# User-tian/Conan

Hardware: AMD Instinct MI355X
Metric: chunks/sec (80 ms chunk, 16 kHz), all streams summed; p50 per-chunk latency beside it (higher is better)
Workload: dtype f32 (3×bf16-limb products, f32 accumulate)

## Files before the change

### conan_amd/csrc/resblock_limb.hip

```cpp
#include <algorithm>
#include <cstring>
#include <type_traits>

#include "kernels.h"

#define RL_MAX_SLOTS 256

#ifndef RL_HELPER_PRIO
#define RL_HELPER_PRIO 3
#endif
#ifndef RL_MATRIX_PRIO
#define RL_MATRIX_PRIO 0
#endif
#ifndef RL_STAMPS
#define RL_STAMPS 0
#endif

#ifdef RL_ABLATE_W
#define RL_WOFF(x) 0
#define RL_WOFF2(a_, b_) (b_)
#else
#define RL_WOFF(x) (x)
#define RL_WOFF2(a_, b_) (a_)
#endif

namespace cnk {

namespace {

typedef float f32x4 __attribute__((ext_vector_type(4)));
typedef __bf16 bf16x8 __attribute__((ext_vector_type(8)));
typedef unsigned short u16;
typedef const f32x4 __attribute__((address_space(1)))* gcf4;
typedef f32x4 __attribute__((address_space(1)))* gf4;
typedef const float __attribute__((address_space(1)))* gcf1;
typedef const int __attribute__((address_space(1)))* gci;

__device__ __forceinline__ f32x4 rl_gload(const void* p) { return *(gcf4)(p); }
__device__ __forceinline__ float4 rl_gload4(const float* p) { const f32x4 v = *(gcf4)(p); return make_float4(v[0], v[1], v[2], v[3]); }
__device__ __forceinline__ void rl_gstore4(float* p, const float4 v) { *(gf4)(p) = (f32x4){v.x, v.y, v.z, v.w}; }

typedef float f32x2 __attribute__((ext_vector_type(2)));
typedef __bf16 bf16x2 __attribute__((ext_vector_type(2)));
__device__ __forceinline__ void rl_split2(const f32x2 x, unsigned& h, unsigned& m, unsigned& l) {
  h = __builtin_bit_cast(unsigned, __builtin_convertvector(x, bf16x2));
  const f32x2 hf = {__uint_as_float(h << 16), __uint_as_float(h & 0xffff0000u)};
  const f32x2 r1 = x - hf;
  m = __builtin_bit_cast(unsigned, __builtin_convertvector(r1, bf16x2));
  const f32x2 mf = {__uint_as_float(m << 16), __uint_as_float(m & 0xffff0000u)};
  const f32x2 r2 = r1 - mf;
  l = __builtin_bit_cast(unsigned, __builtin_convertvector(r2, bf16x2));
}
__device__ __forceinline__ f32x2 rl_lrelu2(const f32x2 x, const float slope) {
  const f32x2 sx = x * slope;
  return (f32x2){__builtin_fmaxf(x[0], sx[0]), __builtin_fmaxf(x[1], sx[1])};
}

template <int C_, int NR2_, int SPAN_>
struct RLGeom {
  static constexpr int C = C_, NR2 = NR2_;
  static constexpr int NR1 = NR2 + 1;
  static constexpr int RO = 16 * NR2;
  static constexpr int XT_ROWS = 16 * NR1;
  static constexpr int MAXSPAN = SPAN_;
  static constexpr int WR_MAX = XT_ROWS + MAXSPAN;
  static constexpr int LDB = C + 16;
  static constexpr int PLW = WR_MAX * LDB;
  static constexpr int PLX = XT_ROWS * LDB;
  static constexpr int LDA = C + 4;
  static constexpr int LDS_U16 = 3 * (PLW + PLX);
  static constexpr int NCT = C / 16;
  static constexpr int NCW = C == 64 ? 1 : 2;
  static constexpr int RSPLIT = 4 / (NCT / NCW);
  static constexpr int NRW1 = (NR1 + RSPLIT - 1) / RSPLIT;
  static constexpr int NRW2 = (NR2 + RSPLIT - 1) / RSPLIT;
  static constexpr int KB = C / 32;
  static constexpr int RING = 2;
  static constexpr int C4 = C / 4;
  static constexpr int BLK = 3 * 512;
  static_assert(C % 32 == 0 && NCT % NCW == 0 && 4 % (NCT / NCW) == 0 && (KB == 1 || KB % RING == 0), "channel count");
  static_assert(RO * LDA * 4 <= 3 * PLX * 2, "accumulator image inside the xt planes");
  static_assert(LDS_U16 * 2 + 32 + 8 * RL_MAX_SLOTS <= 160 * 1024, "LDS budget");
};

template <int NCW, int RING>
__device__ __forceinline__ void rl_prefetch_w(f32x4 (&bw)[RING][NCW][3], const u16* __restrict__ wl, const long long ct_stride) {
#pragma unroll
  for (int q = 0; q < RING; ++q) {
#pragma unroll
    for (int c = 0; c < NCW; ++c)
#pragma unroll
      for (int p = 0; p < 3; ++p) bw[q][c][p] = rl_gload(wl + c * ct_stride + q * 1536 + p * 512);
    __builtin_amdgcn_sched_barrier(0);
  }
}

template <int NRW, int NCW, int LDB, int KB, int RING>
__device__ __forceinline__ void rl_gemm(const u16* __restrict__ src, const int plane, const int row0, const int tap_stride, const int k,
                                        const u16* __restrict__ wl, const long long ct_stride, const u16* __restrict__ wl_next,
                                        const long long ct_stride_next, f32x4 (&acc)[NRW][NCW], f32x4 (&bw)[RING][NCW][3], const int lane) {
  const u16* abase = src + (row0 + (lane & 15)) * LDB + 8 * (lane >> 4);
  f32x4 af[NRW][3];
#pragma unroll
  for (int r = 0; r < NRW; ++r)
#pragma unroll
    for (int p = 0; p < 3; ++p) af[r][p] = *reinterpret_cast<const f32x4*>(abase + p * plane + r * 16 * LDB);
  const int tstep = tap_stride * LDB;
  if constexpr (KB == 1) {
    static_assert(RING == 2, "ring");
    constexpr int PA[6] = {2, 1, 0, 1, 0, 0}, PB[6] = {0, 1, 2, 0, 1, 0};
    auto block = [&](const int j, auto slot_c) __attribute__((always_inline)) {
      constexpr int SL = decltype(slot_c)::value;
      const u16* anext = abase + (j + 1) * tstep;
#pragma unroll
      for (int s = 0; s < 6; ++s)
#pragma unroll
        for (int r = 0; r < NRW; ++r) {
#pragma unroll
          for (int c = 0; c < NCW; ++c)
            acc[r][c] = __builtin_amdgcn_mfma_f32_16x16x32_bf16(__builtin_bit_cast(bf16x8, bw[SL][c][PB[s]]), __builtin_bit_cast(bf16x8, af[r][PA[s]]), acc[r][c], 0, 0, 0);
#ifndef RL_ABLATE_A
          if (s == 0) af[r][2] = *reinterpret_cast<const f32x4*>(anext + 2 * plane + r * 16 * LDB);
          if (s == 3) af[r][1] = *reinterpret_cast<const f32x4*>(anext + plane + r * 16 * LDB);
          if (s == 5) af[r][0] = *reinterpret_cast<const f32x4*>(anext + r * 16 * LDB);
#endif
        }
      const bool own = j + 2 < k;
      const u16* wsrc = own ? wl + (long long)(j + 2) * 1536 : wl_next + (long long)(j + 2 - k) * 1536;
      const long long cs = own ? ct_stride : ct_stride_next;
#pragma unroll
      for (int c = 0; c < NCW; ++c)
#pragma unroll
        for (int p = 0; p < 3; ++p) bw[SL][c][p] = rl_gload(wsrc + c * cs + p * 512);
#pragma unroll
      for (int s = 0; s < 6; ++s) {
        if (s == 0 || s == 3 || s == 5) {
#pragma unroll
          for (int r = 0; r < NRW; ++r) {
            __builtin_amdgcn_sched_group_barrier(0x008, NCW, 0);
            __builtin_amdgcn_sched_group_barrier(0x100, 1, 0);
          }
        } else {
          __builtin_amdgcn_sched_group_barrier(0x008, NRW * NCW, 0);
        }
      }
      __builtin_amdgcn_sched_group_barrier(0x020, 3 * NCW, 0);
    };
    int j = 0;
    for (; j + 1 < k; j += 2) {
      block(j, std::integral_constant<int, 0>{});
      block(j + 1, std::integral_constant<int, 1>{});
    }
    if (j < k) {
      block(j, std::integral_constant<int, 0>{});
#pragma unroll
      for (int c = 0; c < NCW; ++c)
#pragma unroll
        for (int p = 0; p < 3; ++p) { const f32x4 t = bw[0][c][p]; bw[0][c][p] = bw[1][c][p]; bw[1][c][p] = t; }
    }
    return;
  }
  for (int j = 0; j < k; ++j) {
    const u16* arow = abase + j * tstep;
    const bool last = j + 1 == k;
    const u16* wnext = last ? wl_next : wl + (long long)(j + 1) * KB * 1536;
    const long long cnext = last ? ct_stride_next : ct_stride;
#pragma unroll
    for (int q = 0; q < KB; ++q) {
      const u16* anext = (q + 1 < KB) ? arow + (q + 1) * 32 : arow + tstep;
      constexpr int PA[6] = {2, 1, 0, 1, 0, 0}, PB[6] = {0, 1, 2, 0, 1, 0};
#pragma unroll
      for (int s = 0; s < 6; ++s)
#pragma unroll
        for (int r = 0; r < NRW; ++r) {
#pragma unroll
          for (int c = 0; c < NCW; ++c)
            acc[r][c] = __builtin_amdgcn_mfma_f32_16x16x32_bf16(__builtin_bit_cast(bf16x8, bw[q % RING][c][PB[s]]), __builtin_bit_cast(bf16x8, af[r][PA[s]]),
                                                                acc[r][c], 0, 0, 0);
#ifndef RL_ABLATE_A
          if (s == 0) af[r][2] = *reinterpret_cast<const f32x4*>(anext + 2 * plane + r * 16 * LDB);
          if (s == 3) af[r][1] = *reinterpret_cast<const f32x4*>(anext + plane + r * 16 * LDB);
          if (s == 5) af[r][0] = *reinterpret_cast<const f32x4*>(anext + r * 16 * LDB);
#endif
        }
      if (q + RING < KB) {
#pragma unroll
        for (int c = 0; c < NCW; ++c)
#pragma unroll
          for (int p = 0; p < 3; ++p) bw[q % RING][c][p] = rl_gload(wl + RL_WOFF(((long long)j * KB + q + RING) * 1536) + c * ct_stride + p * 512);
      } else {
#pragma unroll
        for (int c = 0; c < NCW; ++c)
#pragma unroll
          for (int p = 0; p < 3; ++p) bw[q % RING][c][p] = rl_gload(RL_WOFF2(wnext, wl) + (q + RING - KB) * 1536 + c * cnext + p * 512);
      }
#pragma unroll
      for (int s = 0; s < 6; ++s) {
        if (s == 0 || s == 3 || s == 5) {
#pragma unroll
          for (int r = 0; r < NRW; ++r) {
            __builtin_amdgcn_sched_group_barrier(0x008, NCW, 0);
            __builtin_amdgcn_sched_group_barrier(0x100, 1, 0);
          }
        } else {
          __builtin_amdgcn_sched_group_barrier(0x008, NRW * NCW, 0);
        }
      }
      __builtin_amdgcn_sched_group_barrier(0x020, 3 * NCW, 0);
      __builtin_amdgcn_sched_barrier(0);
    }
  }
}

}

#define RL_SEL(br_, f) ((br_) == 0 ? a.p[0].f : ((br_) == 1 ? a.p[1].f : a.p[2].f))

template <int C, int NR2, int SPAN, bool MERGE>
__global__ __launch_bounds__(512, 2) void resblock_limb_kernel(const RBArgs a) {
  using G = RLGeom<C, NR2, SPAN>;
  constexpr int LDB = G::LDB;
  __shared__ __attribute__((aligned(16))) u16 lds[G::LDS_U16 + 16 + 4 * RL_MAX_SLOTS];
  u16* const win = lds;
  u16* const xt = lds + 3 * G::PLW;
  float* const accimg = reinterpret_cast<float*>(xt);
  int* const meta = reinterpret_cast<int*>(lds + G::LDS_U16);
  int* const sptab = meta + 8;
  const int tid = threadIdx.x;
  const int lane = tid & 63;
  const int wave = __builtin_amdgcn_readfirstlane(tid >> 6);
  const int ntiles = a.ntiles;
  const float slope = a.slope;
  const int T = a.T;
  constexpr bool merge = MERGE;
  const int np = a.nprob;

  if (wave >= 4) {
    const int ht = tid - 256;
    __builtin_amdgcn_s_setprio(RL_HELPER_PRIO);
    auto hbar = [&]() __attribute__((always_inline)) { asm volatile("s_waitcnt lgkmcnt(0)\n\ts_barrier" ::: "memory"); };
    constexpr int NIT = (G::WR_MAX * G::C4 + 255) / 256;
    float4 wv[NIT];
    int wtotal = 0, wzr = 0;
    auto win_issue = [&](const int p, const int i, const int t0, const int slot, const int pos) __attribute__((always_inline)) {
      const int k = RL_SEL(p, k), d = RL_SEL(p, dil);
      const int wr = G::XT_ROWS + (k - 1) * d;
      const int tw0 = t0 - (k - 1) - (k - 1) * d;
      const int xmode = a.p[0].x.mode, xrate = a.p[0].x.rate;
      const float* xb = RL_SEL(p, x.base) + (long long)(xmode == 0 ? slot : i) * RL_SEL(p, x.slot_stride);
      const unsigned rbase = (xmode == 0 ? (unsigned)pos * (unsigned)xrate : 0u) + (unsigned)(RL_SEL(p, x.off) + tw0);
      const unsigned rmask = xmode == 0 ? (unsigned)RL_SEL(p, x.lmask) : 0xffffffffu;
      wtotal = wr * G::C4;
#pragma unroll
      for (int u = 0; u < NIT; ++u) {
        const int idx = ht + 256 * u;
        const int w = idx / G::C4, c4 = idx - w * G::C4;
        const unsigned row = (rbase + (unsigned)w) & rmask;
        wv[u] = idx < wtotal ? rl_gload4(xb + (long long)row * C + c4 * 4) : make_float4(0.f, 0.f, 0.f, 0.f);
      }
      const long long abs0 = (xmode == 0 ? (long long)pos * xrate : 0ll) + t0 - (k - 1);
      wzr = abs0 >= 0 ? 0 : (abs0 < -(long long)G::XT_ROWS ? G::XT_ROWS : (int)-abs0);
    };
    auto win_write = [&]() __attribute__((always_inline)) {
#pragma unroll
      for (int u = 0; u < NIT; ++u) {
        const int idx = ht + 256 * u;
        const int w = idx / G::C4, c4 = idx - w * G::C4;
        unsigned h[2], m[2], l[2];
        rl_split2(rl_lrelu2((f32x2){wv[u].x, wv[u].y}, slope), h[0], m[0], l[0]);
        rl_split2(rl_lrelu2((f32x2){wv[u].z, wv[u].w}, slope), h[1], m[1], l[1]);
        if (idx < wtotal) {
          u16* dst = win + w * LDB + c4 * 4;
          *reinterpret_cast<uint2*>(dst) = make_uint2(h[0], h[1]);
          *reinterpret_cast<uint2*>(dst + G::PLW) = make_uint2(m[0], m[1]);
          *reinterpret_cast<uint2*>(dst + 2 * G::PLW) = make_uint2(l[0], l[1]);
        }
      }
      if (ht == 0) meta[0] = wzr;
    };
    constexpr int NOUT = (G::RO * G::C4) / 256;
    static_assert((G::RO * G::C4) % 256 == 0 && 256 % G::C4 == 0, "output tile / helper threads");
    const int oc4 = ht % G::C4;
    float4 oacc[NOUT], ores[NOUT], osum[MERGE ? NOUT : 1], ob2 = make_float4(0.f, 0.f, 0.f, 0.f);
    const float* oxb = nullptr; const float* ob2p = nullptr;
    float* oyb = nullptr;
    unsigned oyr0 = 0, oym = 0, oxr0 = 0, oxm = 0;
    int ot0 = 0, op = 0, oyC = C;
#pragma unroll
    for (int u = 0; u < (MERGE ? NOUT : 1); ++u) osum[u] = make_float4(0.f, 0.f, 0.f, 0.f);
    auto out_fetch = [&](const int p, const int i, const int t0, const int slot, const int pos) __attribute__((always_inline)) {
      const int xmode = a.p[0].x.mode, xrate = a.p[0].x.rate, ymode = a.p[0].y.mode, yrate = a.p[0].y.rate;
      oxb = RL_SEL(p, x.base) + (long long)(xmode == 0 ? slot : i) * RL_SEL(p, x.slot_stride);
      oxr0 = (xmode == 0 ? (unsigned)pos * (unsigned)xrate : 0u) + (unsigned)(RL_SEL(p, x.off) + t0);
      oxm = xmode == 0 ? (unsigned)RL_SEL(p, x.lmask) : 0xffffffffu;
      if (!merge) {
        oyb = RL_SEL(p, y.base) + (long long)(ymode == 0 ? slot : i) * RL_SEL(p, y.slot_stride);
        oyr0 = (ymode == 0 ? (unsigned)pos * (unsigned)yrate : 0u) + (unsigned)(RL_SEL(p, y.off) + t0);
        oym = ymode == 0 ? (unsigned)RL_SEL(p, y.lmask) : 0xffffffffu;
      } else {
        const int mmode = a.ymean.mode;
        oyb = a.ymean.base + (long long)(mmode == 0 ? slot : i) * a.ymean.slot_stride;
        oyr0 = (mmode == 0 ? (unsigned)pos * (unsigned)a.ymean.rate : 0u) + (unsigned)(a.ymean.off + t0);
        oym = mmode == 0 ? (unsigned)a.ymean.lmask : 0xffffffffu;
        oyC = a.ymean.C;
      }
      ot0 = t0; op = p;
      ob2p = RL_SEL(p, b2) + oc4 * 4;
#pragma unroll
      for (int u = 0; u < NOUT; ++u) oacc[u] = *reinterpret_cast<const float4*>(accimg + ((ht + 256 * u) / G::C4) * G::LDA + oc4 * 4);
      ob2 = rl_gload4(ob2p);
#pragma unroll
      for (int u = 0; u < NOUT; ++u) {
        const int r = (ht + 256 * u) / G::C4;
        ores[u] = ot0 + r < T ? rl_gload4(oxb + (long long)((oxr0 + (unsigned)r) & oxm) * C + oc4 * 4) : make_float4(0.f, 0.f, 0.f, 0.f);
      }
    };
    auto out_store = [&]() __attribute__((always_inline)) {
#pragma unroll
      for (int u = 0; u < NOUT; ++u) {
        const int r = (ht + 256 * u) / G::C4;
        if (ot0 + r < T) {
          const float4 v = make_float4((oacc[u].x + ob2.x) + ores[u].x, (oacc[u].y + ob2.y) + ores[u].y, (oacc[u].z + ob2.z) + ores[u].z, (oacc[u].w + ob2.w) + ores[u].w);
          if constexpr (!MERGE) rl_gstore4(oyb + (long long)((oyr0 + (unsigned)r) & oym) * C + oc4 * 4, v);
          else {
            float4 sm = osum[MERGE ? u : 0];
            if (op == 0) sm = v; else { sm.x += v.x; sm.y += v.y; sm.z += v.z; sm.w += v.w; }
            osum[MERGE ? u : 0] = sm;
            if (op == np - 1) {
              const float dn = (float)np;
              if (np > 1) { sm.x /= dn; sm.y /= dn; sm.z /= dn; sm.w /= dn; }
              sm.x = sm.x > 0.f ? sm.x : sm.x * slope; sm.y = sm.y > 0.f ? sm.y : sm.y * slope;
              sm.z = sm.z > 0.f ? sm.z : sm.z * slope; sm.w = sm.w > 0.f ? sm.w : sm.w * slope;
              rl_gstore4(oyb + (long long)((oyr0 + (unsigned)r) & oym) * oyC + oc4 * 4, sm);
            }
          }
        }
      }
    };
#if RL_STAMPS
    const unsigned long long h_t0 = __builtin_amdgcn_s_memtime();
    unsigned long long h_t[6] = {0, 0, 0, 0, 0, 0};
#define RL_HT(i_) h_t[i_] = __builtin_amdgcn_s_memtime() - h_t0
#else
#define RL_HT(i_)
#endif
    int dv0 = 0;
    if (wave == 4 && lane == 0) dv0 = __hip_atomic_fetch_add(a.sched, 1, __ATOMIC_RELAXED, __HIP_MEMORY_SCOPE_AGENT);
    for (int e = ht; e < a.n; e += 256) {
      const int sl = a.slots ? *(gci)(a.slots + e) : e;
      sptab[2 * e] = sl; sptab[2 * e + 1] = a.pos ? *(gci)(a.pos + sl) : 0;
    }
    const int tps = a.tiles_per_slot, per_prob = a.n * tps;
    auto decode = [&](const int e, int& p, int& i, int& t0) __attribute__((always_inline)) {
      if constexpr (!MERGE) {
        const int b = e / per_prob, rem = e - b * per_prob;
        p = b == 0 ? a.order[0] : (b == 1 ? a.order[1] : a.order[2]);
        i = rem / tps; t0 = (rem - i * tps) * G::RO;
      } else {
        const int g = e / np;
        p = e - g * np; i = g / tps; t0 = (g - i * tps) * G::RO;
      }
    };
    int cur = -1, p = -1, i = 0, t0 = 0;
    if (wave == 4) {
      cur = __builtin_amdgcn_readfirstlane(dv0) * (merge ? np : 1);
      if (cur >= ntiles) cur = -1;
      if (cur >= 0) decode(cur, p, i, t0);
      if (lane == 0) { meta[1] = cur; meta[2] = p; meta[3] = 0; }
    }
    RL_HT(0);
    asm volatile("s_waitcnt lgkmcnt(0)\n\ts_barrier" ::: "memory");
    RL_HT(1);
    if (wave != 4) {
      cur = __builtin_amdgcn_readfirstlane(meta[1]);
      if (cur >= 0) decode(cur, p, i, t0);
    }
    if (cur >= 0) {
    int slot = __builtin_amdgcn_readfirstlane(sptab[2 * i]), pos = __builtin_amdgcn_readfirstlane(sptab[2 * i + 1]);
    win_issue(p, i, t0, slot, pos);
    RL_HT(2);
    int gen = 1;
    int dv = 0, dnext = -1;
    auto draw_issue = [&](const int have, const int idx_prev, const int p_prev) __attribute__((always_inline)) {
      if (wave == 4 && lane == 0 && have) {
        if (merge && p_prev != np - 1) dnext = idx_prev + 1;
        else { dnext = -1; dv = __hip_atomic_fetch_add(a.sched, 1, __ATOMIC_RELAXED, __HIP_MEMORY_SCOPE_AGENT); }
      }
    };
    auto draw_take = [&](const int have) __attribute__((always_inline)) {
      int idx = -1;
      if (!have) return idx;
      if (wave == 4) {
        const int drawn = dv * (merge ? np : 1);
        idx = __builtin_amdgcn_readfirstlane(dnext >= 0 ? dnext : drawn);
        if (idx >= ntiles) idx = -1;
        if (lane == 0) {
          meta[1] = idx;
          asm volatile("s_waitcnt lgkmcnt(0)" ::: "memory");
          __hip_atomic_store(&meta[3], gen, __ATOMIC_RELEASE, __HIP_MEMORY_SCOPE_WORKGROUP);
        }
      } else {
        while (__hip_atomic_load(&meta[3], __ATOMIC_ACQUIRE, __HIP_MEMORY_SCOPE_WORKGROUP) != gen) __builtin_amdgcn_s_sleep(4);
        idx = __builtin_amdgcn_readfirstlane(meta[1]);
      }
      ++gen;
      return idx;
    };
    const bool deep = ntiles >= 5 * (int)gridDim.x * (merge ? np : 1);
    auto stage = [&](const int e) __attribute__((always_inline)) {
      int pe, ie, te;
      decode(e, pe, ie, te);
      win_issue(pe, ie, te, __builtin_amdgcn_readfirstlane(sptab[2 * ie]), __builtin_amdgcn_readfirstlane(sptab[2 * ie + 1]));
      return pe;
    };
    int nxt = -1, pn = -1;
    if (deep) {
      draw_issue(1, cur, p);
      nxt = draw_take(1);
    }
    RL_HT(3);
    win_write();
    RL_HT(4);
    hbar();
    RL_HT(5);
#if RL_STAMPS
    if (a.dbg && blockIdx.x == 0 && wave == 4 && lane == 0) { unsigned long long* q = a.dbg + 256 * 4 + 12; for (int e = 0; e < 6; ++e) q[e] = h_t[e]; }
#endif
    bool pending = false;
    for (;;) {
      const bool have = deep ? nxt >= 0 : true;
      if (deep && nxt >= 0) pn = stage(nxt);
      draw_issue(have, deep ? nxt : cur, deep ? pn : p);
      if (pending) out_store();
      int nn = -1;
      if (!deep) {
        nxt = draw_take(have); pn = -1;
        if (nxt >= 0) pn = stage(nxt);
      }
      if (ht == 0) meta[2] = nxt >= 0 ? pn : -1;
      hbar();
      hbar();
      if (nxt >= 0) win_write();
      hbar();
      hbar();
      out_fetch(p, i, t0, slot, pos);
      pending = true;
      if (deep) nn = draw_take(have);
      if (nxt < 0) break;
      cur = nxt;
      decode(cur, p, i, t0);
      slot = __builtin_amdgcn_readfirstlane(sptab[2 * i]); pos = __builtin_amdgcn_readfirstlane(sptab[2 * i + 1]);
      nxt = nn;
    }
    if (pending) out_store();
    }
    if (ht == 0) {
      const int d = __hip_atomic_fetch_add(a.sched + 1, 1, __ATOMIC_RELAXED, __HIP_MEMORY_SCOPE_AGENT);
      if (d == (int)gridDim.x - 1) {
        __hip_atomic_store(a.sched, 0, __ATOMIC_RELAXED, __HIP_MEMORY_SCOPE_AGENT);
        __hip_atomic_store(a.sched + 1, 0, __ATOMIC_RELAXED, __HIP_MEMORY_SCOPE_AGENT);
      }
    }
    return;
  }

  if (RL_MATRIX_PRIO) __builtin_amdgcn_s_setprio(RL_MATRIX_PRIO);
  auto bar = [&]() __attribute__((always_inline)) { asm volatile("s_waitcnt lgkmcnt(0)\n\ts_barrier" ::: "memory"); };
  const int wc = wave % (4 / G::RSPLIT);
  const int wr = wave / (4 / G::RSPLIT);
  const int ct0 = wc * G::NCW;
  const int lr = lane & 15, lg = lane >> 4;
#if RL_STAMPS
  unsigned long long st_gemm = 0, st_t0 = __builtin_amdgcn_s_memtime(), st_r0 = __builtin_amdgcn_s_memrealtime(), st_bar = 0, st_b3 = 0, st_b1 = 0, st_b4 = 0, st_b2 = 0, st_e1 = 0, st_e2 = 0, st_tiles = 0, st_head = 0, st_pre = 0, st_mid = 0;
#define RL_T() __builtin_amdgcn_s_memtime()
#define RL_BAR(acc_) do { const unsigned long long q0_ = RL_T(); bar(); const unsigned long long q1_ = RL_T(); acc_ += q1_ - q0_; st_bar += q1_ - q0_; } while (0)
#define RL_GEMM(...) do { const unsigned long long s0_ = RL_T(); __VA_ARGS__; asm volatile("s_nop 0" ::"v"(acc[0][0][0])); st_gemm += RL_T() - s0_; } while (0)
#else
#define RL_BAR(acc_) bar()
#define RL_GEMM(...) __VA_ARGS__
#endif
  f32x4 bw[G::RING][G::NCW][3];
  bar();
  int p = __builtin_amdgcn_readfirstlane(meta[2]);
  if (p < 0) return;
  {
    const long long cs = (long long)(RL_SEL(p, k) + 1) * G::KB * G::BLK;
    rl_prefetch_w<G::NCW, G::RING>(bw, RL_SEL(p, w1l) + (long long)ct0 * cs + lane * 8, cs);
  }
  bar();
#if RL_STAMPS
  st_head = RL_T() - st_t0;
#endif
  while (p >= 0) {
#if RL_STAMPS
    const unsigned long long top_ = RL_T();
#endif
    const int k = RL_SEL(p, k), d = RL_SEL(p, dil);
    const u16* const w1 = RL_SEL(p, w1l);
    const u16* const w2 = RL_SEL(p, w2l);
    const float* const b1 = RL_SEL(p, b1);
    const long long ct_stride = (long long)(k + 1) * G::KB * G::BLK;
    const int zrows = __builtin_amdgcn_readfirstlane(meta[0]);
    f32x4 b1v[G::NCW];
#pragma unroll
    for (int c = 0; c < G::NCW; ++c) b1v[c] = rl_gload(b1 + (ct0 + c) * 16 + 4 * lg);
    int pn;
    {
      f32x4 acc[G::NRW1][G::NCW];
#pragma unroll
      for (int r = 0; r < G::NRW1; ++r)
#pragma unroll
        for (int c = 0; c < G::NCW; ++c) acc[r][c] = (f32x4){0.f, 0.f, 0.f, 0.f};
      const int rt0 = wr * G::NRW1;
#if RL_STAMPS
      st_pre += RL_T() - top_;
#endif
      RL_GEMM(rl_gemm<G::NRW1, G::NCW, LDB, G::KB, G::RING>(win, G::PLW, rt0 * 16, d, k, w1 + (long long)ct0 * ct_stride + lane * 8, ct_stride,
                                                           w2 + (long long)ct0 * ct_stride + lane * 8, ct_stride, acc, bw, lane));
      RL_BAR(st_b3);
#if RL_STAMPS
      const unsigned long long e1_0 = RL_T();
#endif
      auto epilogue1 = [&](auto zr_c) __attribute__((always_inline)) {
        constexpr bool ZR = decltype(zr_c)::value;
#pragma unroll
        for (int c = 0; c < G::NCW; ++c) {
          const int col = (ct0 + c) * 16 + 4 * lg;
#pragma unroll
          for (int r = 0; r < G::NRW1; ++r) {
            if (rt0 + r < G::NR1) {
              const int m = (rt0 + r) * 16 + lr;
              unsigned h[2], mm[2], l[2];
              const f32x4 v = acc[r][c] + b1v[c];
              rl_split2(rl_lrelu2((f32x2){v[0], v[1]}, slope), h[0], mm[0], l[0]);
              rl_split2(rl_lrelu2((f32x2){v[2], v[3]}, slope), h[1], mm[1], l[1]);
              const bool zr = ZR && m < zrows;
              u16* dst = xt + m * LDB + col;
              *reinterpret_cast<uint2*>(dst) = zr ? make_uint2(0u, 0u) : make_uint2(h[0], h[1]);
              *reinterpret_cast<uint2*>(dst + G::PLX) = zr ? make_uint2(0u, 0u) : make_uint2(mm[0], mm[1]);
              *reinterpret_cast<uint2*>(dst + 2 * G::PLX) = zr ? make_uint2(0u, 0u) : make_uint2(l[0], l[1]);
            }
          }
        }
      };
      if (zrows > 0) epilogue1(std::true_type{}); else epilogue1(std::false_type{});
#if RL_STAMPS
      asm volatile("s_waitcnt lgkmcnt(0)" ::: "memory"); st_e1 += RL_T() - e1_0; ++st_tiles;
#endif
    }
    RL_BAR(st_b1);
#if RL_STAMPS
    const unsigned long long mid_ = RL_T();
#endif
    pn = __builtin_amdgcn_readfirstlane(meta[2]);
    const int pnx = pn >= 0 ? pn : p;
    const long long csn = (long long)(RL_SEL(pnx, k) + 1) * G::KB * G::BLK;
    const u16* const w1n = RL_SEL(pnx, w1l) + (long long)ct0 * csn + lane * 8;
    {
      f32x4 acc[G::NRW2][G::NCW];
#pragma unroll
      for (int r = 0; r < G::NRW2; ++r)
#pragma unroll
        for (int c = 0; c < G::NCW; ++c) acc[r][c] = (f32x4){0.f, 0.f, 0.f, 0.f};
      const int rt0 = wr * G::NRW2;
#if RL_STAMPS
      st_mid += RL_T() - mid_;
#endif
      RL_GEMM(rl_gemm<G::NRW2, G::NCW, LDB, G::KB, G::RING>(xt, G::PLX, rt0 * 16, 1, k, w2 + (long long)ct0 * ct_stride + lane * 8, ct_stride,
                                                           w1n, csn, acc, bw, lane));
      RL_BAR(st_b4);
#if RL_STAMPS
      const unsigned long long e2_0 = RL_T();
#endif
#pragma unroll
      for (int c = 0; c < G::NCW; ++c) {
        const int col = (ct0 + c) * 16 + 4 * lg;
#pragma unroll
        for (int r = 0; r < G::NRW2; ++r) {
          if (rt0 + r < NR2) *reinterpret_cast<f32x4*>(accimg + ((rt0 + r) * 16 + lr) * G::LDA + col) = acc[r][c];
        }
      }
#if RL_STAMPS
      asm volatile("s_waitcnt lgkmcnt(0)" ::: "memory"); st_e2 += RL_T() - e2_0;
#endif
    }
    RL_BAR(st_b2);
    p = pn;
  }
#if RL_STAMPS
  if (a.dbg && tid == 0) {
    unsigned long long* o = a.dbg + blockIdx.x * 4;
    if (blockIdx.x == 0) { unsigned long long* q = a.dbg + 256 * 4; q[0] = st_b3; q[1] = st_b1; q[2] = st_b4; q[3] = st_b2; q[4] = st_e1; q[5] = st_e2; q[6] = st_tiles; q[7] = st_gemm; q[8] = __builtin_amdgcn_s_memtime() - st_t0; q[9] = st_head; q[10] = st_pre; q[11] = st_mid; }
    o[0] = st_gemm; o[1] = __builtin_amdgcn_s_memtime() - st_t0; o[2] = __builtin_amdgcn_s_memrealtime() - st_r0; o[3] = st_bar;
  }
#endif
}


namespace {
struct RLCand { int C, NR2, span; };
const RLCand kLimbCands[] = {{32, 10, 50}, {64, 5, 50}, {128, 2, 50}};
}

bool resblock_limb_supported(int C, int kmax, int span_max) {
  for (const RLCand& c : kLimbCands)
    if (c.C == C && span_max <= c.span) return kmax <= 16;
  return false;
}

int resblock_limb_rows(int C, int span_max) {
  int best = 0;
  for (const RLCand& c : kLimbCands)
    if (c.C == C && span_max <= c.span) best = std::max(best, 16 * c.NR2);
  return best;
}

template <int C, int NR2, int SPAN, bool MERGE = false>
static bool launch_rl(const RBArgs& ain, int num_cu, hipStream_t st) {
  RBArgs a = ain;
  const int ro = 16 * NR2;
  a.tiles_per_slot = (a.T + ro - 1) / ro;
  const int total = a.nprob * a.n * a.tiles_per_slot;
  if (total <= 0) return true;
  if (!a.sched) return false;
  for (int p = 0; p < a.nprob; ++p) if (!a.p[p].w1l || !a.p[p].w2l) return false;
  if (a.n > RL_MAX_SLOTS) return false;
  if (!(a.slope > 0.f && a.slope <= 1.f)) return false;
  for (int p = 0; p < 3; ++p) a.order[p] = p;
  std::stable_sort(a.order, a.order + a.nprob, [&](int x, int y) { return a.p[x].k > a.p[y].k; });
  const int grid = std::min(a.merge ? total / a.nprob : total, num_cu);
  a.tiles = nullptr; a.ntiles = total;
  hipLaunchKernelGGL((resblock_limb_kernel<C, NR2, SPAN, MERGE>), dim3(grid), dim3(512), 0, st, a);
  return true;
}

bool launch_resblock_limb(const RBArgs& a, int C, int rows, int num_cu, hipStream_t st) {
  const int nr2 = rows / 16;
  if (a.merge) {
    if (C == 32 && nr2 == 10) return launch_rl<32, 10, 50, true>(a, num_cu, st);
    if (C == 64 && nr2 == 5) return launch_rl<64, 5, 50, true>(a, num_cu, st);
    if (C == 128 && nr2 == 2) return launch_rl<128, 2, 50, true>(a, num_cu, st);
    return false;
  }
  if (C == 32 && nr2 == 10) return launch_rl<32, 10, 50>(a, num_cu, st);
  if (C == 64 && nr2 == 5) return launch_rl<64, 5, 50>(a, num_cu, st);
  if (C == 128 && nr2 == 2) return launch_rl<128, 2, 50>(a, num_cu, st);
  return false;
}

bool resblock_limb_can_merge(int C, int rows) { return (C == 32 && rows == 160) || (C == 64 && rows == 80) || (C == 128 && rows == 32); }

const char* resblock_limb_name(int C, int rows, bool merge) {
  static thread_local char buf[72];
  const int span = 50;
  snprintf(buf, sizeof(buf), "cnk::resblock_limb_kernel<%d, %d, %d, %s>", C, rows / 16, span, merge ? "true" : "false");
  return buf;
}

}
```

Measured before the change: 47640.

## Deepen weight prefetch ring to three slots for C=128 non-merged resblock GEMMs

For C=128 without merging, the register ring holding prefetched bf16-limb weight fragments grows from two to three slots. That lets weight global loads run further ahead of the MFMAs that consume them. Because KB (4) is not a multiple of 3, the tap loop is unrolled by three with rotating slot offsets, and the hand-off of the last tap's prefetch to the next GEMM is adjusted. Weight loads switch to scalar base pointers plus a per-lane byte offset, and a vmcnt wait is added before each GEMM so the ring has landed. The extra ring slot raises VGPR pressure and the explicit waits could stall.

```diff
diff --git a/conan_amd/csrc/resblock_limb.hip b/conan_amd/csrc/resblock_limb.hip
--- a/conan_amd/csrc/resblock_limb.hip
+++ b/conan_amd/csrc/resblock_limb.hip
@@ -56,7 +56,7 @@
   return (f32x2){__builtin_fmaxf(x[0], sx[0]), __builtin_fmaxf(x[1], sx[1])};
 }
 
-template <int C_, int NR2_, int SPAN_>
+template <int C_, int NR2_, int SPAN_, bool MERGE_ = false>
 struct RLGeom {
   static constexpr int C = C_, NR2 = NR2_;
   static constexpr int NR1 = NR2 + 1;
@@ -75,10 +75,10 @@
   static constexpr int NRW1 = (NR1 + RSPLIT - 1) / RSPLIT;
   static constexpr int NRW2 = (NR2 + RSPLIT - 1) / RSPLIT;
   static constexpr int KB = C / 32;
-  static constexpr int RING = 2;
+  static constexpr int RING = (C == 128 && !MERGE_) ? 3 : 2;
   static constexpr int C4 = C / 4;
   static constexpr int BLK = 3 * 512;
-  static_assert(C % 32 == 0 && NCT % NCW == 0 && 4 % (NCT / NCW) == 0 && (KB == 1 || KB % RING == 0), "channel count");
+  static_assert(C % 32 == 0 && NCT % NCW == 0 && 4 % (NCT / NCW) == 0 && (KB == 1 ? RING == 2 : RING <= KB), "channel count");
   static_assert(RO * LDA * 4 <= 3 * PLX * 2, "accumulator image inside the xt planes");
   static_assert(LDS_U16 * 2 + 32 + 8 * RL_MAX_SLOTS <= 160 * 1024, "LDS budget");
 };
@@ -93,6 +93,11 @@
       for (int p = 0; p < 3; ++p) bw[q][c][p] = rl_gload(wl + c * ct_stride + q * 1536 + p * 512);
     __builtin_amdgcn_sched_barrier(0);
   }
+}
+
+template <int KB, int RING>
+__device__ __forceinline__ void rl_ring_landed() {
+  if constexpr (KB != 1 && KB % RING != 0) __builtin_amdgcn_s_waitcnt(0x0f70);
 }
 
 template <int NRW, int NCW, int LDB, int KB, int RING>
@@ -160,13 +165,25 @@
     }
     return;
   }
-  for (int j = 0; j < k; ++j) {
+  constexpr bool WUNI = KB != 1 && KB % RING != 0;
+  const unsigned wlane = (unsigned)lane * 16u;
+  auto wload = [&](const u16* ptr, const int limb) __attribute__((always_inline)) {
+    if constexpr (WUNI) {
+      asm("" : "+s"(ptr));
+      return *(gcf4)(reinterpret_cast<const char*>(ptr) + wlane + limb * 1024);
+    } else {
+      return rl_gload(ptr + limb * 512);
+    }
+  };
+  auto tap = [&](const int j, auto s0_c) __attribute__((always_inline)) {
+    constexpr int S0 = decltype(s0_c)::value;
     const u16* arow = abase + j * tstep;
     const bool last = j + 1 == k;
     const u16* wnext = last ? wl_next : wl + (long long)(j + 1) * KB * 1536;
     const long long cnext = last ? ct_stride_next : ct_stride;
 #pragma unroll
     for (int q = 0; q < KB; ++q) {
+      const int SL = (S0 + q) % RING;
       const u16* anext = (q + 1 < KB) ? arow + (q + 1) * 32 : arow + tstep;
       constexpr int PA[6] = {2, 1, 0, 1, 0, 0}, PB[6] = {0, 1, 2, 0, 1, 0};
 #pragma unroll
@@ -175,7 +192,7 @@
         for (int r = 0; r < NRW; ++r) {
 #pragma unroll
           for (int c = 0; c < NCW; ++c)
-            acc[r][c] = __builtin_amdgcn_mfma_f32_16x16x32_bf16(__builtin_bit_cast(bf16x8, bw[q % RING][c][PB[s]]), __builtin_bit_cast(bf16x8, af[r][PA[s]]),
+            acc[r][c] = __builtin_amdgcn_mfma_f32_16x16x32_bf16(__builtin_bit_cast(bf16x8, bw[SL][c][PB[s]]), __builtin_bit_cast(bf16x8, af[r][PA[s]]),
                                                                 acc[r][c], 0, 0, 0);
 #ifndef RL_ABLATE_A
           if (s == 0) af[r][2] = *reinterpret_cast<const f32x4*>(anext + 2 * plane + r * 16 * LDB);
@@ -183,16 +200,17 @@
           if (s == 5) af[r][0] = *reinterpret_cast<const f32x4*>(anext + r * 16 * LDB);
 #endif
         }
+      const int hand = (WUNI && last) ? SL : q + RING - KB;
       if (q + RING < KB) {
 #pragma unroll
         for (int c = 0; c < NCW; ++c)
 #pragma unroll
-          for (int p = 0; p < 3; ++p) bw[q % RING][c][p] = rl_gload(wl + RL_WOFF(((long long)j * KB + q + RING) * 1536) + c * ct_stride + p * 512);
+          for (int p = 0; p < 3; ++p) bw[SL][c][p] = wload(wl + RL_WOFF(((long long)j * KB + q + RING) * 1536) + c * ct_stride, p);
       } else {
 #pragma unroll
         for (int c = 0; c < NCW; ++c)
 #pragma unroll
-          for (int p = 0; p < 3; ++p) bw[q % RING][c][p] = rl_gload(RL_WOFF2(wnext, wl) + (q + RING - KB) * 1536 + c * cnext + p * 512);
+          for (int p = 0; p < 3; ++p) bw[SL][c][p] = wload(RL_WOFF2(wnext, wl) + hand * 1536 + c * cnext, p);
       }
 #pragma unroll
       for (int s = 0; s < 6; ++s) {
@@ -209,6 +227,24 @@
       __builtin_amdgcn_sched_group_barrier(0x020, 3 * NCW, 0);
       __builtin_amdgcn_sched_barrier(0);
     }
+  };
+  using S0 = std::integral_constant<int, 0>;
+  if constexpr (KB == 1 || KB % RING == 0) {
+    for (int j = 0; j < k; ++j) tap(j, S0{});
+  } else {
+    static_assert(RING == 3 && KB % RING == 1, "ring");
+    using S1 = std::integral_constant<int, 1>;
+    using S2 = std::integral_constant<int, 2>;
+    int j = 0;
+    for (; j + 3 <= k; j += 3) {
+      tap(j, S0{});
+      tap(j + 1, S1{});
+      tap(j + 2, S2{});
+    }
+    if (j < k) {
+      tap(j, S0{});
+      if (j + 1 < k) tap(j + 1, S1{});
+    }
   }
 }
 
@@ -218,7 +254,7 @@
 
 template <int C, int NR2, int SPAN, bool MERGE>
 __global__ __launch_bounds__(512, 2) void resblock_limb_kernel(const RBArgs a) {
-  using G = RLGeom<C, NR2, SPAN>;
+  using G = RLGeom<C, NR2, SPAN, MERGE>;
   constexpr int LDB = G::LDB;
   __shared__ __attribute__((aligned(16))) u16 lds[G::LDS_U16 + 16 + 4 * RL_MAX_SLOTS];
   u16* const win = lds;
@@ -480,6 +516,7 @@
 #define RL_GEMM(...) __VA_ARGS__
 #endif
   f32x4 bw[G::RING][G::NCW][3];
+  const int wl8 = (G::KB != 1 && G::KB % G::RING != 0) ? 0 : lane * 8;
   bar();
   int p = __builtin_amdgcn_readfirstlane(meta[2]);
   if (p < 0) return;
@@ -501,6 +538,7 @@
     const float* const b1 = RL_SEL(p, b1);
     const long long ct_stride = (long long)(k + 1) * G::KB * G::BLK;
     const int zrows = __builtin_amdgcn_readfirstlane(meta[0]);
+    rl_ring_landed<G::KB, G::RING>();
     f32x4 b1v[G::NCW];
 #pragma unroll
     for (int c = 0; c < G::NCW; ++c) b1v[c] = rl_gload(b1 + (ct0 + c) * 16 + 4 * lg);
@@ -515,8 +553,8 @@
 #if RL_STAMPS
       st_pre += RL_T() - top_;
 #endif
-      RL_GEMM(rl_gemm<G::NRW1, G::NCW, LDB, G::KB, G::RING>(win, G::PLW, rt0 * 16, d, k, w1 + (long long)ct0 * ct_stride + lane * 8, ct_stride,
-                                                           w2 + (long long)ct0 * ct_stride + lane * 8, ct_stride, acc, bw, lane));
+      RL_GEMM(rl_gemm<G::NRW1, G::NCW, LDB, G::KB, G::RING>(win, G::PLW, rt0 * 16, d, k, w1 + (long long)ct0 * ct_stride + wl8, ct_stride,
+                                                           w2 + (long long)ct0 * ct_stride + wl8, ct_stride, acc, bw, lane));
       RL_BAR(st_b3);
 #if RL_STAMPS
       const unsigned long long e1_0 = RL_T();
@@ -553,9 +591,10 @@
     const unsigned long long mid_ = RL_T();
 #endif
     pn = __builtin_amdgcn_readfirstlane(meta[2]);
+    rl_ring_landed<G::KB, G::RING>();
     const int pnx = pn >= 0 ? pn : p;
     const long long csn = (long long)(RL_SEL(pnx, k) + 1) * G::KB * G::BLK;
-    const u16* const w1n = RL_SEL(pnx, w1l) + (long long)ct0 * csn + lane * 8;
+    const u16* const w1n = RL_SEL(pnx, w1l) + (long long)ct0 * csn + wl8;
     {
       f32x4 acc[G::NRW2][G::NCW];
 #pragma unroll
@@ -566,7 +605,7 @@
 #if RL_STAMPS
       st_mid += RL_T() - mid_;
 #endif
-      RL_GEMM(rl_gemm<G::NRW2, G::NCW, LDB, G::KB, G::RING>(xt, G::PLX, rt0 * 16, 1, k, w2 + (long long)ct0 * ct_stride + lane * 8, ct_stride,
+      RL_GEMM(rl_gemm<G::NRW2, G::NCW, LDB, G::KB, G::RING>(xt, G::PLX, rt0 * 16, 1, k, w2 + (long long)ct0 * ct_stride + wl8, ct_stride,
                                                            w1n, csn, acc, bw, lane));
       RL_BAR(st_b4);
 #if RL_STAMPS
```

Result: no change. 48110, median of 6 (+1.0%).
